# matheusfalcaopinto/triple-hybrid-rag

Hardware: AMD Instinct MI355X
Metric: queries/sec (fused top-10) (higher is better)
Workload: dtype f16 MFMA shortlist scan (f32 accumulate) + f64 rescoring of the f32 rows; 1 GPU; 1000000-doc / 768-d dense-only brute-force cosine top-10 (BASELINE.json configs[1]); pipeline=dense, docs=1000000, dim=768, semantic_top_k=100, fused_top_k=10, shortlist=f16, parallelism=single GPU, world_size_seen=1, rescued_queries=0

## Files before the change

triple-hybrid-rag_amd/_native.py:

```python
from __future__ import annotations

import ctypes as C
import os
from typing import Optional, Tuple

import torch

from . import _build

THR_FLAG_CERTIFIED = 1
THR_FLAG_OVERFLOW = 2
THR_FLAG_EXACT = 4
THR_DENSE_MAX_K = 256
THR_BM25_MAX_TERMS = 32
THR_BM25_MAX_QUERIES = 1 << 20
THR_GRAPH_MAX_SEEDS = 16
THR_RRF_MAX_PER_CHANNEL = 128
THR_TOPK_MAX = 128
THR_SCOPE_MAX_COLS = 8
THR_SCOPE_MAX_PREDS = 4096
THR_SCOPE_MAX_QUERIES = 1 << 20
ABI_VERSION = 9

_lib = None
# ... 92 lines not shown
        except AttributeError as e:
            raise NativeError(f"{path} does not export {name}") from e
        fn.restype, fn.argtypes = res, args
    if lib.thr_abi_version() != ABI_VERSION:
        raise NativeError("libthr_hip.so ABI version mismatch; rebuild")
    _lib = lib
    return lib


def _check(rc: int, what: str) -> None:
    if rc != 0:
        msg = load().thr_error_string(rc).decode()
        raise NativeError(f"{what} failed: {msg} (code {rc})")


def _stream() -> int:
    return torch.cuda.current_stream().cuda_stream


def _dev(t: Optional[torch.Tensor], dtype, name: str, ndim: Optional[int] = None) -> int:
    if t is None:
        return 0
    if not isinstance(t, torch.Tensor) or not t.is_cuda:
        raise NativeError(f"{name}: expected a CUDA(HIP) tensor")
    if t.dtype != dtype:
        raise NativeError(f"{name}: expected dtype {dtype}, got {t.dtype}")
    if not t.is_contiguous():
        raise NativeError(f"{name}: must be contiguous")
    if ndim is not None and t.dim() != ndim:
        raise NativeError(f"{name}: expected {ndim} dims, got {t.dim()}")
    return t.data_ptr()


def device_info() -> Tuple[int, int, str]:
    cus, hbm = C.c_int(0), C.c_int64(0)
    arch = C.create_string_buffer(128)
    torch.cuda.current_device()
    _check(load().thr_device_info(C.byref(cus), C.byref(hbm), arch, 128), "thr_device_info")
    return cus.value, hbm.value, arch.value.decode()


def embed_postproc(full: torch.Tensor, store_dim: int) -> torch.Tensor:
    p = _dev(full, torch.float32, "full", 2)
    n, fd = full.shape
    out = torch.empty((n, min(fd, store_dim)), dtype=torch.float32, device=full.device)
    if n:
        _check(load().thr_embed_postproc(p, n, fd, store_dim, out.data_ptr(), _stream()),
               "thr_embed_postproc")
    return out


def doc_norms(docs: torch.Tensor) -> Tuple[torch.Tensor, torch.Tensor]:
    p = _dev(docs, torch.float32, "docs", 2)
    n, d = docs.shape
    dn = torch.empty(n, dtype=torch.float64, device=docs.device)
    inv = torch.empty(n, dtype=torch.float32, device=docs.device)
    if n:
        _check(load().thr_doc_norms(p, n, d, dn.data_ptr(), inv.data_ptr(), _stream()),
               "thr_doc_norms")
    return dn, inv


def dense_workspace_bytes(n_docs: int, dim: int, n_queries: int, kprime: int) -> int:
    return int(load().thr_dense_workspace_bytes(n_docs, dim, n_queries, kprime))


def _alloc_out(nq: int, k: int, device):
    tile = torch.empty((2, nq, k), dtype=torch.int64, device=device)
    return (tile[0].view(torch.float64), tile[1],
            torch.empty(nq, dtype=torch.int32, device=device),
            torch.empty(nq, dtype=torch.int32, device=device))


def _coll(doc_coll, query_coll, n: int, nq: int):
    if query_coll is None:
        return None, None
    if doc_coll is None:
        raise NativeError("query_coll without doc_coll")
    if doc_coll.shape != (n,) or query_coll.shape != (nq,):
        raise NativeError("doc_coll / query_coll have the wrong length")
    return _dev(doc_coll, torch.int32, "doc_coll", 1), _dev(query_coll, torch.int32, "query_coll", 1)


def dense_topk(docs, dnorm, inv_norm, queries, k: int, kprime: int, id_base: int = 0,
               workspace: Optional[torch.Tensor] = None, doc_coll=None, query_coll=None):
    pd = _dev(docs, torch.float32, "docs", 2)
    n, d = docs.shape
    pq = _dev(queries, torch.float32, "queries", 2)
    nq = queries.shape[0]
    if queries.shape[1] != d:
        raise NativeError(f"queries dim {queries.shape[1]} != docs dim {d}")
    pn = _dev(dnorm, torch.float64, "dnorm", 1)
    pi = _dev(inv_norm, torch.float32, "inv_norm", 1)
    if dnorm.shape[0] != n or inv_norm.shape[0] != n:
        raise NativeError("dnorm / inv_norm length != n_docs")
    need = dense_workspace_bytes(n, d, nq, kprime)
    if workspace is None or workspace.numel() * workspace.element_size() < need:
        workspace = torch.empty(need, dtype=torch.uint8, device=docs.device)
    pw = _dev(workspace, workspace.dtype, "workspace")
    S, I, cnt, flg = _alloc_out(nq, k, docs.device)
    pdc, pqc = _coll(doc_coll, query_coll, n, nq)
    _check(load().thr_dense_topk(pd, pn, pi, n, d, id_base, pq, nq, k, kprime, pdc, pqc, S.data_ptr(),
                                 I.data_ptr(), cnt.data_ptr(), flg.data_ptr(), pw,
                                 workspace.numel() * workspace.element_size(), _stream()),
           "thr_dense_topk")
    return S, I, cnt, flg


def dense_topk_exact(docs, dnorm, queries, k: int, id_base: int = 0, doc_coll=None, query_coll=None):
    pd = _dev(docs, torch.float32, "docs", 2)
    n, d = docs.shape
    pq = _dev(queries, torch.float32, "queries", 2)
    nq = queries.shape[0]
    if queries.shape[1] != d:
        raise NativeError(f"queries dim {queries.shape[1]} != docs dim {d}")
    pn = _dev(dnorm, torch.float64, "dnorm", 1)
    if dnorm.shape[0] != n:
        raise NativeError("dnorm length != n_docs")
    need = int(load().thr_dense_exact_workspace_bytes(n, nq))
    ws = torch.empty(need, dtype=torch.uint8, device=docs.device)
    S, I, cnt, flg = _alloc_out(nq, k, docs.device)
    pdc, pqc = _coll(doc_coll, query_coll, n, nq)
    _check(load().thr_dense_topk_exact(pd, pn, n, d, id_base, pq, nq, k, pdc, pqc, S.data_ptr(),
                                       I.data_ptr(), cnt.data_ptr(), flg.data_ptr(),
                                       ws.data_ptr(), need, _stream()), "thr_dense_topk_exact")
    return S, I, cnt, flg


def dense_scan_probe(docs, inv_norm, queries, workspace: torch.Tensor) -> None:
    pd = _dev(docs, torch.float32, "docs", 2)
    n, d = docs.shape
    pq = _dev(queries, torch.float32, "queries", 2)
    if queries.shape[1] != d or inv_norm.shape[0] != n:
        raise NativeError("probe: shape mismatch")
    pi = _dev(inv_norm, torch.float32, "inv_norm", 1)
    pw = _dev(workspace, workspace.dtype, "workspace")
    _check(load().thr_dense_scan_probe(pd, pi, n, d, pq, queries.shape[0], pw,
                                       workspace.numel() * workspace.element_size(), _stream()),
           "thr_dense_scan_probe")


def dense_f16_query_tile(dim: int, packed: bool, n_queries: int) -> int:
    return int(load().thr_dense_f16_query_tile(dim, 1 if packed else 0, n_queries))


def dense_f16_max_queries(dim: int, packed: bool) -> int:
    return int(load().thr_dense_f16_max_queries(dim, 1 if packed else 0))


def dense_rescue_workspace_bytes(n_queries: int, k: int) -> int:
    return int(load().thr_dense_rescue_workspace_bytes(n_queries, k))


def dense_rescue(docs, dnorm, queries, S, I, cnt, flg, id_base: int = 0,
                 workspace: Optional[torch.Tensor] = None, doc_coll=None, query_coll=None) -> torch.Tensor:
    pd = _dev(docs, torch.float32, "docs", 2)
    pn = _dev(dnorm, torch.float64, "dnorm", 1)
    pq = _dev(queries, torch.float32, "queries", 2)
    n, d = docs.shape
    nq, k = I.shape
    need = int(load().thr_dense_rescue_workspace_bytes(nq, k))
    if workspace is None or workspace.numel() * workspace.element_size() < need:
        workspace = torch.empty(need, dtype=torch.uint8, device=docs.device)
    n_rescued = torch.zeros(1, dtype=torch.int32, device=docs.device)
    pdc, pqc = _coll(doc_coll, query_coll, n, nq)
    _check(load().thr_dense_rescue(pd, pn, n, d, id_base, pq, nq, k, pdc, pqc, S.data_ptr(), I.data_ptr(),
                                   cnt.data_ptr(), flg.data_ptr(), n_rescued.data_ptr(),
                                   workspace.data_ptr(),
                                   workspace.numel() * workspace.element_size(), _stream()),
           "thr_dense_rescue")
    return n_rescued


def dense_quantize_f16(docs: torch.Tensor, keep_copy: bool = True):
    p = _dev(docs, torch.float32, "docs", 2)
    n, d = docs.shape
    d16 = None
    if keep_copy:
        nbytes = int(load().thr_dense_f16_copy_bytes(n, d))
        d16 = torch.empty((nbytes // (2 * d), d), dtype=torch.float16, device=docs.device)
    err = torch.zeros(1, dtype=torch.float32, device=docs.device)
    _check(load().thr_dense_quantize_f16(p, n, d, d16.data_ptr() if keep_copy else None,
                                         err.data_ptr(), _stream()), "thr_dense_quantize_f16")
    return d16, float(err.item())


def dense_quantize_f16_into(docs: torch.Tensor, d16: Optional[torch.Tensor], err: torch.Tensor) -> None:
    p = _dev(docs, torch.float32, "docs", 2)
    n, d = docs.shape
    pe = _dev(err, torch.float32, "err", 1)
    ph = None
    if d16 is not None:
        ph = _dev(d16, torch.float16, "d16", 2)
        if d16.shape[1] != d or d16.numel() * 2 < int(load().thr_dense_f16_copy_bytes(n, d)):
            raise NativeError("dense_quantize_f16_into: the float16 destination is too small")
    if err.numel() != 1:
        raise NativeError("dense_quantize_f16_into: err is one float32")
    _check(load().thr_dense_quantize_f16(p, n, d, ph, pe, _stream()), "thr_dense_quantize_f16")


def dense_f16_layout(dim: int) -> str:
    return f"fragment-major/mfma{32 if os.environ.get('THR_DENSE_MFMA') == '32' else 16}/dim{dim}"


def dense_f16_workspace_bytes(n_docs: int, dim: int, n_queries: int, kprime: int) -> int:
    return int(load().thr_dense_f16_workspace_bytes(n_docs, dim, n_queries, kprime))


def dense_topk_f16(docs, docs16, doc_rel_err: float, dnorm, inv_norm, queries, k: int,
                   kprime: int, id_base: int = 0, workspace: Optional[torch.Tensor] = None,
                   doc_coll=None, query_coll=None):
    pd = _dev(docs, torch.float32, "docs", 2)
    ph = _dev(docs16, torch.float16, "docs16", 2) if docs16 is not None else None
    n, d = docs.shape
    if docs16 is not None and tuple(docs16.shape) != ((n + 31) // 32 * 32, d):
        raise NativeError("docs16 is not the fragment-major copy of docs (thr_dense_quantize_f16)")
    pq = _dev(queries, torch.float32, "queries", 2)
    nq = queries.shape[0]
    if queries.shape[1] != d:
        raise NativeError(f"queries dim {queries.shape[1]} != docs dim {d}")
    pn = _dev(dnorm, torch.float64, "dnorm", 1)
    pi = _dev(inv_norm, torch.float32, "inv_norm", 1)
    if dnorm.shape[0] != n or inv_norm.shape[0] != n:
        raise NativeError("dnorm / inv_norm length != n_docs")
    need = dense_f16_workspace_bytes(n, d, nq, kprime)
    if workspace is None or workspace.numel() * workspace.element_size() < need:
        workspace = torch.empty(need, dtype=torch.uint8, device=docs.device)
    pw = _dev(workspace, workspace.dtype, "workspace")
    S, I, cnt, flg = _alloc_out(nq, k, docs.device)
    pdc, pqc = _coll(doc_coll, query_coll, n, nq)
    _check(load().thr_dense_topk_f16(pd, ph, float(doc_rel_err), pn, pi, n, d, id_base, pq, nq, k,
                                     kprime, pdc, pqc, S.data_ptr(), I.data_ptr(), cnt.data_ptr(),
                                     flg.data_ptr(), pw,
                                     workspace.numel() * workspace.element_size(), _stream()),
           "thr_dense_topk_f16")
    return S, I, cnt, flg


def dense_shortlist_f16(docs, docs16, doc_rel_err: float, inv_norm, queries, kprime: int, m: int,
                        workspace: torch.Tensor, doc_coll=None, query_coll=None) -> torch.Tensor:
    pd = _dev(docs, torch.float32, "docs", 2)
    ph = _dev(docs16, torch.float16, "docs16", 2) if docs16 is not None else None
    n, d = docs.shape
    pq = _dev(queries, torch.float32, "queries", 2)
    nq = queries.shape[0]
    if queries.shape[1] != d or inv_norm.shape[0] != n:
        raise NativeError("shortlist: shape mismatch")
    pi = _dev(inv_norm, torch.float32, "inv_norm", 1)
    need = dense_f16_workspace_bytes(n, d, nq, kprime)
    if workspace.numel() * workspace.element_size() < need:
        raise NativeError("shortlist: workspace smaller than thr_dense_f16_workspace_bytes")
    pw = _dev(workspace, workspace.dtype, "workspace")
    pdc, pqc = _coll(doc_coll, query_coll, n, nq)
    lb = torch.empty((nq, m), dtype=torch.float32, device=docs.device)
    _check(load().thr_dense_shortlist_f16(pd, ph, float(doc_rel_err), pi, n, d, pq, nq, kprime, pdc, pqc,
                                          m, lb.data_ptr(), pw,
                                          workspace.numel() * workspace.element_size(), _stream()),
           "thr_dense_shortlist_f16")
    return lb


def dense_floor(top_lb: torch.Tensor, k: int) -> torch.Tensor:
    p = _dev(top_lb, torch.float32, "top_lb", 3)
    g, nq, m = top_lb.shape
    out = torch.empty(nq, dtype=torch.float32, device=top_lb.device)
    _check(load().thr_dense_floor(p, g, nq, m, k, out.data_ptr(), _stream()), "thr_dense_floor")
    return out


def dense_finish_f16(docs, docs16, doc_rel_err: float, dnorm, inv_norm, queries, k: int, kprime: int,
                     gfloor: Optional[torch.Tensor], id_base: int, workspace: torch.Tensor,
                     doc_coll=None, query_coll=None, lb_all: Optional[torch.Tensor] = None):
    pd = _dev(docs, torch.float32, "docs", 2)
    ph = _dev(docs16, torch.float16, "docs16", 2) if docs16 is not None else None
    n, d = docs.shape
    pq = _dev(queries, torch.float32, "queries", 2)
    nq = queries.shape[0]
    pn = _dev(dnorm, torch.float64, "dnorm", 1)
    pi = _dev(inv_norm, torch.float32, "inv_norm", 1)
    if queries.shape[1] != d or dnorm.shape[0] != n or inv_norm.shape[0] != n:
        raise NativeError("finish: shape mismatch")
    pg = None
    if gfloor is not None:
        pg = _dev(gfloor, torch.float32, "gfloor", 1)
        if gfloor.shape[0] != nq:
            raise NativeError("gfloor: one value per query")
    pl, g, m = None, 0, 0
    if lb_all is not None:
        if gfloor is not None:
            raise NativeError("finish: gfloor or lb_all, not both")
        pl = _dev(lb_all, torch.float32, "lb_all", 3)
        g, nq_l, m = lb_all.shape
        if nq_l != nq:
            raise NativeError("lb_all: [n_shards, nq, m]")
    pw = _dev(workspace, workspace.dtype, "workspace")
    S, I, cnt, flg = _alloc_out(nq, k, docs.device)
    pdc, pqc = _coll(doc_coll, query_coll, n, nq)
    _check(load().thr_dense_finish_f16(pd, ph, float(doc_rel_err), pn, pi, n, d, id_base, pq, nq, k,
                                       kprime, pdc, pqc, pg, pl, g, m, S.data_ptr(), I.data_ptr(),
                                       cnt.data_ptr(), flg.data_ptr(), pw,
                                       workspace.numel() * workspace.element_size(), _stream()),
           "thr_dense_finish_f16")
    return S, I, cnt, flg


def dense_scan_probe_f16(docs, docs16, inv_norm, queries, workspace: torch.Tensor) -> None:
    pd = _dev(docs, torch.float32, "docs", 2)
    ph = _dev(docs16, torch.float16, "docs16", 2) if docs16 is not None else None
    n, d = docs.shape
    pq = _dev(queries, torch.float32, "queries", 2)
    if queries.shape[1] != d or inv_norm.shape[0] != n:
        raise NativeError("probe: shape mismatch")
    pi = _dev(inv_norm, torch.float32, "inv_norm", 1)
    pw = _dev(workspace, workspace.dtype, "workspace")
    _check(load().thr_dense_scan_probe_f16(pd, ph, pi, n, d, pq, queries.shape[0], pw,
                                           workspace.numel() * workspace.element_size(),
                                           _stream()), "thr_dense_scan_probe_f16")
# ... 508 lines not shown
```

triple-hybrid-rag_amd/csrc/dense.hip:

```cpp
#include <stdlib.h>

#include "dense_common.hpp"

namespace thr {

struct DenseKnobs {
    bool forced_q;
    int shape;
    bool forced32;
};
static const DenseKnobs& dense_knobs() {
    static const DenseKnobs knobs = [] {
        DenseKnobs K;
        const char* e = getenv("THR_DENSE_F16");
        K.forced_q = e && e[0] == 'q';
        e = getenv("THR_DENSE_MFMA");
        K.shape = (e && atoi(e) == 32) ? 32 : 16;
        e = getenv("THR_DENSE_QW");
        K.forced32 = e && atoi(e) == 32;
        return K;
    }();
    return knobs;
}

bool qreg_staggered(int dim) { return !dense_knobs().forced_q && dim <= 768; }
int qreg_waves(int dim) { return qreg_staggered(dim) ? 8 : 4; }
int qreg_shape(int) { return dense_knobs().shape; }
int qreg_qw(int dim) {
    return (dim == 1024 && !qreg_staggered(dim) && qreg_shape(dim) == 16 && !dense_knobs().forced32) ? 48 : 32;
}
constexpr int QREG_MAX_SEG = 1024;
int qreg_max_queries(int dim) {
    const int qt = qreg_qw(dim) * qreg_waves(dim);
    const int64_t m = (int64_t)UINT32_MAX / ((int64_t)CAND_CAP * (int64_t)sizeof(Cand));
    return (int)(m / qt * qt);
}


static DensePlan make_plan(void* ws, int64_t n_docs, int n_queries, int kprime, int kind, int dim,
                           bool packed) {
    DensePlan p;
    p.kind = kind;
    p.packed = kind == KIND_F16 && packed;
    p.nq = (kind == KIND_F16 && !p.packed) ? f16_pick_nq(dim) : 1;
    p.row_bits = (kind == KIND_F16 && !p.packed) ? ROW_BITS_F16 : ROW_BITS;
    p.qtile = p.packed ? qreg_qw(dim) * qreg_waves(dim)
              : kind == KIND_F16 ? 32 * p.nq : MF_QT;
    p.ntiles = (n_queries + p.qtile - 1) / p.qtile;
    p.qpad = p.ntiles * p.qtile;
    const int64_t groups = (n_docs + MF_ROWS - 1) / MF_ROWS;
    p.sampled = n_docs > CAND_CAP / 2;
    const int ks_cap = p.packed ? 32 : 64;
    p.ksample = kprime < ks_cap ? kprime : ks_cap;
    double aim = (p.packed ? 2896.0 : 4096.0) * sqrt((double)n_docs / 1.0e6);
    const double aim_lo = 8.0 * kprime < 4096.0 ? 8.0 * kprime : 4096.0;
    aim = aim < aim_lo ? aim_lo : aim > 4096.0 ? 4096.0 : aim;
    int64_t target = (int64_t)((double)n_docs * (double)p.ksample / aim);
    if (target > SAMPLE_MAX) target = SAMPLE_MAX;
    if (target < 4 * (int64_t)p.ksample) target = 4 * (int64_t)p.ksample;
    int64_t sg = (target + MF_ROWS - 1) / MF_ROWS;
    if (sg > groups) sg = groups;
    p.sample_stride = sg > 0 ? groups / sg : 1;
    if (p.sample_stride < 1) p.sample_stride = 1;
    p.sample_groups = p.sampled ? sg : 0;
    p.sample_docs = p.sample_groups * MF_ROWS;
    p.groups = groups;
    p.tile_cap = p.packed ? 1 : p.qtile * (CAND_CAP / 2);
    const size_t qpad = (size_t)p.qpad;
    Arena A{(char*)ws};
    p.tau = A.take<float>(qpad);
    p.qerr = A.take<float>(qpad);
    if (kind != KIND_F16) p.qerr = nullptr;
    p.cnt = A.take<int>(qpad * (p.packed ? QREG_MAX_SEG : 1));
    p.tcnt = A.take<int>(p.ntiles);
    p.cand = A.take<Cand>(qpad * CAND_CAP);
    p.tlist = A.take<Cand>((size_t)p.ntiles * p.tile_cap);
    p.sample = A.take<float>(qpad * (size_t)p.sample_docs);
    p.qfrag = A.take<_Float16>(p.packed ? qpad * (size_t)dim : 0);
    p.sel_rows = A.take<int32_t>(qpad * SEL_BIG_BAND);
    p.sel_meta = A.take<int32_t>(4 * qpad);
    p.total = A.total;
    return p;
}

dim3 scan_grid(int ntiles, int64_t n_row_tiles, int waves, bool* shared_rows, int blocks_per_cu,
               int m_cap) {
    const int cus = num_cus() * blocks_per_cu;
    int64_t m_max = n_row_tiles / (8 * (int64_t)waves);
    if (m_max < 1) m_max = 1;
    if (m_max > m_cap) m_max = m_cap;
    int best_m = 1;
    double best_eff = 0.0;
    for (int m = 1; m <= (int)m_max; ++m) {
        const int64_t g = 8 * (int64_t)m * ntiles;
        const int64_t rounds = (g + cus - 1) / cus;
        const double eff = (double)g / (double)(rounds * cus);
        if (eff > best_eff + 1e-9) {
            best_eff = eff;
            best_m = m;
        }
    }
    *shared_rows = ntiles > 1;
    return dim3((unsigned)(8 * best_m * ntiles), 1u);
}

bool scan_nt(bool shared_rows) { return !shared_rows; }


template <int MODE>
static int launch_scan(const DensePlan& P, const DenseIndex& X, const DenseBatch& B, int* nseg = nullptr) {
    constexpr bool all = MODE == MODE_ALL;
    const int64_t units = all ? P.sample_groups : P.groups, stride = all ? P.sample_stride : 1;
    const float* tau = all ? nullptr : P.tau;
    float* smp = all ? P.sample : nullptr;
    const int64_t ld = all ? P.sample_docs : 0;
    const int32_t* doc_coll = all ? nullptr : X.doc_coll;
    const int32_t* query_coll = all ? nullptr : B.query_coll;
    if (P.packed)
        return launch_scan_f16q<MODE>(X.dim, X.docs16, P.qfrag, P.ntiles, units, stride, tau,
                                      all ? nullptr : P.cnt, all ? nullptr : P.cand, smp, ld, B.st,
                                      nseg, doc_coll, query_coll, B.n_queries);
    int* tcnt = all ? nullptr : P.tcnt;
    Cand* tlist = all ? nullptr : P.tlist;
    const int tile_cap = all ? 0 : P.tile_cap;
    if (P.kind == KIND_F16)
        return launch_scan_f16<MODE>(X.dim, P.nq, X.docs, X.inv_norm, X.n_docs, B.queries, B.n_queries,
                                     P.ntiles, units, stride, tau, tcnt, tlist, tile_cap, smp, ld, B.st,
                                     doc_coll, query_coll);
    return launch_scan_mfma<MODE>(X.dim, X.docs, X.inv_norm, X.n_docs, B.queries, B.n_queries, P.ntiles,
                                  units, stride, tau, tcnt, tlist, tile_cap, smp, ld, B.st, doc_coll,
                                  query_coll);
}

static int dense_pipeline(const DensePlan& P, const DenseIndex& X, const DenseBatch& B,
                          const DensePhase& S) {
    int rc, nseg = 0;
    if (S.phase != PIPE_FINISH) {
        hipError_t e = hipMemsetAsync(P.cnt, 0, (char*)P.cand - (char*)P.cnt, B.st);
        if (e != hipSuccess) return (int)e;
        if (P.packed && (rc = launch_pack_queries(X.dim, B.queries, B.n_queries, P.qpad, P.qfrag, P.qerr, B.st)))
            return rc;
        if (P.sampled && (rc = launch_scan<MODE_ALL>(P, X, B))) return rc;
        if ((rc = launch_threshold(P, X, B))) return rc;
        if ((rc = launch_scan<MODE_FILTER>(P, X, B, &nseg))) return rc;
        if (!P.packed && (rc = launch_bucket(P, B.st))) return rc;
    } else if (P.packed) {
        if ((rc = launch_scan_f16q<MODE_FILTER, true>(X.dim, X.docs16, P.qfrag, P.ntiles, P.groups, 1,
                                                      nullptr, nullptr, nullptr, nullptr, 0, B.st, &nseg)))
            return rc;
    }
    if ((rc = launch_band(P, X, B, S, nseg))) return rc;
    if (S.phase == PIPE_SHORTLIST) return THR_OK;
    return launch_rescore(P, X, B);
}

}

using namespace thr;

extern "C" size_t thr_dense_workspace_bytes(int64_t n_docs, int dim, int n_queries, int kprime) {
    if (n_docs <= 0 || n_queries <= 0) return 0;
    return make_plan(nullptr, n_docs, n_queries, kprime, KIND_F32, dim, false).total;
}

static int dense_args_ok(const void* docs, const void* dnorm, const void* inv_norm,
                         const void* queries, const void* a, const void* b, const void* c,
                         const void* d, const void* ws, int64_t n_docs, int n_queries, int k,
                         int kprime) {
    THR_RETURN_IF(!docs || !dnorm || !inv_norm || !queries || !a || !b || !c || !d || !ws,
                  THR_ERR_INVALID);
    THR_RETURN_IF(n_docs <= 0 || n_queries <= 0 || k <= 0 || kprime < k ||
                      kprime > THR_DENSE_MAX_K,
                  THR_ERR_INVALID);
    return THR_OK;
}

extern "C" int thr_dense_topk(const float* docs, const double* dnorm, const float* inv_norm,
                              int64_t n_docs, int dim, int64_t id_base, const float* queries,
                              int n_queries, int k, int kprime, const int32_t* doc_coll,
                              const int32_t* query_coll, double* out_scores,
                              int64_t* out_ids, int32_t* out_counts, uint32_t* out_flags,
                              void* workspace, size_t workspace_bytes, thr_stream_t stream) {
    clear_status();
    int rc = dense_args_ok(docs, dnorm, inv_norm, queries, out_scores, out_ids, out_counts,
                           out_flags, workspace, n_docs, n_queries, k, kprime);
    if (rc) return rc;
    THR_RETURN_IF((query_coll != nullptr) != (doc_coll != nullptr), THR_ERR_INVALID);
    THR_RETURN_IF(dim <= 0 || dim % CHUNK != 0 || dim / CHUNK > 4, THR_ERR_UNSUPPORTED);
    THR_RETURN_IF(n_docs >= (int64_t)1 << ROW_BITS, THR_ERR_UNSUPPORTED);
    const DensePlan P = make_plan(workspace, n_docs, n_queries, kprime, KIND_F32, dim, false);
    THR_RETURN_IF(workspace_bytes < P.total, THR_ERR_WORKSPACE);
    const DenseIndex X{docs, inv_norm, n_docs, dim, dnorm, id_base, doc_coll};
    const DenseBatch B{queries, n_queries, k, kprime, query_coll, (hipStream_t)stream,
                       out_scores, out_ids, out_counts, out_flags};
    return dense_pipeline(P, X, B, DensePhase{});
}

extern "C" size_t thr_dense_f16_workspace_bytes(int64_t n_docs, int dim, int n_queries,
                                                int kprime) {
    if (n_docs <= 0 || n_queries <= 0) return 0;
    const size_t a = make_plan(nullptr, n_docs, n_queries, kprime, KIND_F16, dim, false).total;
    const size_t b = make_plan(nullptr, n_docs, n_queries, kprime, KIND_F16, dim, true).total;
    return a > b ? a : b;
}

extern "C" int thr_dense_f16_max_queries(int dim, int packed) {
    if (dim != 512 && dim != 768 && dim != 1024) return 0;
    return packed ? qreg_max_queries(dim) : INT32_MAX;
}

extern "C" int thr_dense_f16_query_tile(int dim, int packed, int n_queries) {
    if (dim != 512 && dim != 768 && dim != 1024) return 0;
    (void)n_queries;
    return packed ? qreg_qw(dim) * qreg_waves(dim) : 32 * f16_pick_nq(dim);
}

extern "C" size_t thr_dense_f16_copy_bytes(int64_t n_docs, int dim) {
    if (n_docs <= 0 || dim <= 0) return 0;
    return sizeof(_Float16) * (size_t)((n_docs + 31) / 32 * 32) * (size_t)dim;
}

extern "C" int thr_dense_quantize_f16(const float* docs, int64_t n_docs, int dim, uint16_t* docs16,
                                      float* max_rel_err, thr_stream_t stream) {
    clear_status();
    THR_RETURN_IF(!docs || !max_rel_err || n_docs <= 0 || dim <= 0, THR_ERR_INVALID);
    THR_RETURN_IF(dim % 64 != 0, THR_ERR_UNSUPPORTED);
    hipStream_t st = (hipStream_t)stream;
    hipError_t e = hipMemsetAsync(max_rel_err, 0, sizeof(float), st);
    if (e != hipSuccess) return (int)e;
    return launch_quantize_f16(docs, n_docs, dim, reinterpret_cast<_Float16*>(docs16),
                               reinterpret_cast<unsigned int*>(max_rel_err), st);
}

static int f16_args_ok(const float* docs, const uint16_t* docs16, double doc_rel_err, int64_t n_docs,
                       int dim, int n_queries, const int32_t* doc_coll, const int32_t* query_coll) {
    (void)docs;
    THR_RETURN_IF((query_coll != nullptr) != (doc_coll != nullptr), THR_ERR_INVALID);
    THR_RETURN_IF(!(doc_rel_err >= 0.0) || !(doc_rel_err < 1.0), THR_ERR_INVALID);
    THR_RETURN_IF(dim != 512 && dim != 768 && dim != 1024, THR_ERR_UNSUPPORTED);
    THR_RETURN_IF(n_docs >= (int64_t)1 << ROW_BITS_F16, THR_ERR_UNSUPPORTED);
    THR_RETURN_IF(docs16 != nullptr && n_queries > qreg_max_queries(dim), THR_ERR_UNSUPPORTED);
    return THR_OK;
}


extern "C" int thr_dense_topk_f16(const float* docs, const uint16_t* docs16, double doc_rel_err,
                                  const double* dnorm, const float* inv_norm, int64_t n_docs,
                                  int dim, int64_t id_base, const float* queries, int n_queries,
                                  int k, int kprime, const int32_t* doc_coll,
                                  const int32_t* query_coll, double* out_scores, int64_t* out_ids,
                                  int32_t* out_counts, uint32_t* out_flags, void* workspace,
                                  size_t workspace_bytes, thr_stream_t stream) {
    clear_status();
    int rc = dense_args_ok(docs, dnorm, inv_norm, queries, out_scores, out_ids, out_counts,
                           out_flags, workspace, n_docs, n_queries, k, kprime);
    if (rc) return rc;
    if ((rc = f16_args_ok(docs, docs16, doc_rel_err, n_docs, dim, n_queries, doc_coll, query_coll))) return rc;
    const DensePlan P = make_plan(workspace, n_docs, n_queries, kprime, KIND_F16, dim, docs16 != nullptr);
    THR_RETURN_IF(workspace_bytes < P.total, THR_ERR_WORKSPACE);
    const DenseIndex X{docs, inv_norm, n_docs, dim, dnorm, id_base, doc_coll,
                       reinterpret_cast<const _Float16*>(docs16), doc_rel_err};
    const DenseBatch B{queries, n_queries, k, kprime, query_coll, (hipStream_t)stream,
                       out_scores, out_ids, out_counts, out_flags};
    return dense_pipeline(P, X, B, DensePhase{});
}

extern "C" int thr_dense_shortlist_f16(const float* docs, const uint16_t* docs16, double doc_rel_err,
                                       const float* inv_norm, int64_t n_docs, int dim,
                                       const float* queries, int n_queries, int kprime,
                                       const int32_t* doc_coll, const int32_t* query_coll, int m,
                                       float* top_lb, void* workspace, size_t workspace_bytes,
                                       thr_stream_t stream) {
    clear_status();
    THR_RETURN_IF(!docs || !inv_norm || !queries || !top_lb || !workspace, THR_ERR_INVALID);
    THR_RETURN_IF(n_docs <= 0 || n_queries <= 0 || kprime <= 0 || kprime > THR_DENSE_MAX_K || m <= 0 ||
                      m > THR_DENSE_MAX_K,
                  THR_ERR_INVALID);
    int rc = f16_args_ok(docs, docs16, doc_rel_err, n_docs, dim, n_queries, doc_coll, query_coll);
    if (rc) return rc;
    const DensePlan P = make_plan(workspace, n_docs, n_queries, kprime, KIND_F16, dim, docs16 != nullptr);
    THR_RETURN_IF(workspace_bytes < P.total, THR_ERR_WORKSPACE);
    const DenseIndex X{docs, inv_norm, n_docs, dim, nullptr, 0, doc_coll,
                       reinterpret_cast<const _Float16*>(docs16), doc_rel_err};
    const DenseBatch B{queries, n_queries, 0, kprime, query_coll, (hipStream_t)stream};
    return dense_pipeline(P, X, B, DensePhase{PIPE_SHORTLIST, top_lb, m});
}

extern "C" int thr_dense_finish_f16(const float* docs, const uint16_t* docs16, double doc_rel_err,
                                    const double* dnorm, const float* inv_norm, int64_t n_docs,
                                    int dim, int64_t id_base, const float* queries, int n_queries,
                                    int k, int kprime, const int32_t* doc_coll,
                                    const int32_t* query_coll, const float* gfloor,
// ... 81 lines not shown
```

triple-hybrid-rag_amd/csrc/rrf.hip:

```cpp
#include "thr_common.hpp"

namespace thr {

constexpr int RRF_THREADS = 128;
constexpr int RRF_MAXC = THR_RRF_MAX_PER_CHANNEL;
constexpr int RRF_SLOTS = 512;

__device__ __forceinline__ int last_rank(const int64_t* l, int n, int64_t id) {
    int r = 0;
    for (int j = 0; j < n; ++j)
        if (l[j] == id) r = j + 1;
    return r;
}
__device__ __forceinline__ bool seen_before(const int64_t* l, int i, int64_t id) {
    for (int j = 0; j < i; ++j)
        if (l[j] == id) return true;
    return false;
}

constexpr int RRF_RAG2 = 0, RRF_STANDALONE = 1, RRF_TWO = 2;
__device__ __forceinline__ int occurrences(const int64_t* l, int n, int64_t id) {
    int c = 0;
    for (int j = 0; j < n; ++j) c += l[j] == id ? 1 : 0;
    return c;
}

template <int MODE>
__global__ __launch_bounds__(RRF_THREADS) void rrf_fuse_kernel(
    const int64_t* __restrict__ lex, int n_lex, const int64_t* __restrict__ sem, int n_sem,
    const int64_t* __restrict__ gra, int n_gra, double w_lex, double w_sem, double w_gra, int rrf_k,
    int top_k, int64_t* __restrict__ out_ids, double* __restrict__ out_scores,
    int32_t* __restrict__ out_ranks, int32_t* __restrict__ out_counts) {
    static_assert(RRF_THREADS == RRF_MAXC && RRF_THREADS == 2 * WAVE, "one thread per position");
    __shared__ int64_t L[3][RRF_MAXC];
    __shared__ int len[3];
    __shared__ int wave_new[3][2];
    __shared__ double s_s[RRF_SLOTS];
    __shared__ int64_t c_id[RRF_SLOTS];
    __shared__ int c_rank[RRF_SLOTS][3];
    __shared__ int order[RRF_SLOTS];

    const int q = blockIdx.x, t = threadIdx.x, lane = t & 63, wave = t >> 6;
    const int64_t* src[3] = {lex, sem, gra};
    const int width[3] = {lex ? n_lex : 0, sem ? n_sem : 0, gra ? n_gra : 0};
    if (t < 3) len[t] = width[t];
    __syncthreads();
    for (int ch = 0; ch < 3; ++ch) {
        const int64_t id = t < width[ch] ? src[ch][(int64_t)q * width[ch] + t] : -1;
        L[ch][t] = id;
        if (t < width[ch] && id < 0) atomicMin(&len[ch], t);
    }
    __syncthreads();

    bool nw[3];
    int within[3];
    for (int ch = 0; ch < 3; ++ch) {
        nw[ch] = false;
        if (t < len[ch]) {
            const int64_t id = L[ch][t];
            nw[ch] = !seen_before(L[ch], t, id);
            for (int e = 0; e < ch && nw[ch]; ++e)
                if (last_rank(L[e], len[e], id)) nw[ch] = false;
        }
        const uint64_t m = __ballot(nw[ch]);
        within[ch] = __popcll(m & ((1ull << lane) - 1ull));
        if (lane == 0) wave_new[ch][wave] = __popcll(m);
    }
    __syncthreads();
    int base = 0, n = 0;
    for (int ch = 0; ch < 3; ++ch) {
        const int here = base + (wave ? wave_new[ch][0] : 0) + within[ch];
        base += wave_new[ch][0] + wave_new[ch][1];
        if (!nw[ch]) continue;
        const int64_t id = L[ch][t];
        const int lr = last_rank(L[0], len[0], id);
        const int sr = last_rank(L[1], len[1], id);
        const int gr = last_rank(L[2], len[2], id);
        double score = 0.0;
        if (MODE == RRF_RAG2) {
            if (lr) score = __dadd_rn(score, __ddiv_rn(w_lex, (double)(rrf_k + lr)));
            if (sr) score = __dadd_rn(score, __ddiv_rn(w_sem, (double)(rrf_k + sr)));
            if (gr) score = __dadd_rn(score, __ddiv_rn(w_gra, (double)(rrf_k + gr)));
        } else {
            const double w[3] = {w_lex, w_sem, w_gra};
            const int rk[3] = {lr, sr, gr};
#pragma unroll
            for (int c = 0; c < 3; ++c)
                if (rk[c]) {
                    const double v = __dmul_rn(w[c], __ddiv_rn(1.0, (double)(rrf_k + rk[c])));
                    const int reps = (MODE == RRF_TWO && c == 0) ? 1 : occurrences(L[c], len[c], id);
                    for (int r = 0; r < reps; ++r) score = __dadd_rn(score, v);
                }
        }
        c_id[here] = id;
        c_rank[here][0] = lr;
        c_rank[here][1] = sr;
        c_rank[here][2] = gr;
        s_s[here] = score;
    }
    n = base;
    __syncthreads();
    for (int p = t; p < n; p += RRF_THREADS) {
        const double ms = s_s[p];
        int rank = 0;
        for (int j = 0; j < n; ++j) {
            const double o = s_s[j];
            rank += (o > ms || (o == ms && j < p)) ? 1 : 0;
        }
        order[rank] = p;
    }
    __syncthreads();
    for (int i = t; i < top_k; i += RRF_THREADS) {
        const bool ok = i < n;
        const int p = ok ? order[i] : 0;
        out_ids[(int64_t)q * top_k + i] = ok ? c_id[p] : -1;
        out_scores[(int64_t)q * top_k + i] = ok ? s_s[p] : -INFINITY;
        if (out_ranks)
            for (int c = 0; c < 3; ++c)
                out_ranks[((int64_t)q * top_k + i) * 3 + c] = ok ? c_rank[p][c] : 0;
    }
    if (t == 0) out_counts[q] = n < top_k ? n : top_k;
}

__global__ __launch_bounds__(RRF_THREADS) void rerank_order_kernel(
    const float* __restrict__ scores, int n_lists, int64_t list_stride,
    const int64_t* __restrict__ ids, const int32_t* __restrict__ counts, int n, int top_k,
    int64_t* __restrict__ out_ids, double* __restrict__ out_scores, int32_t* __restrict__ out_counts) {
    __shared__ double s_s[RRF_SLOTS];
    __shared__ int order[RRF_SLOTS];
    const int q = blockIdx.x, t = threadIdx.x;
    int cnt = counts ? counts[q] : n;
    cnt = cnt < n ? cnt : n;
    for (int p = t; p < cnt; p += RRF_THREADS) {
        float best = -INFINITY;
        for (int l = 0; l < n_lists; ++l) best = fmaxf(best, scores[(int64_t)l * list_stride + (int64_t)q * n + p]);
        s_s[p] = best > -INFINITY ? (double)best : 0.0;
    }
    __syncthreads();
    for (int p = t; p < cnt; p += RRF_THREADS) {
        const double ms = s_s[p];
        int rank = 0;
        for (int j = 0; j < cnt; ++j) {
            const double o = s_s[j];
            rank += (o > ms || (o == ms && j < p)) ? 1 : 0;
        }
        order[rank] = p;
    }
    __syncthreads();
    for (int i = t; i < top_k; i += RRF_THREADS) {
        const bool ok = i < cnt;
        const int p = ok ? order[i] : 0;
        out_ids[(int64_t)q * top_k + i] = ok ? ids[(int64_t)q * n + p] : -1;
        out_scores[(int64_t)q * top_k + i] = ok ? s_s[p] : -INFINITY;
    }
    if (t == 0) out_counts[q] = cnt < top_k ? cnt : top_k;
}

__global__ __launch_bounds__(RRF_THREADS) void fuse_post_kernel(
    const int64_t* __restrict__ ids, const double* __restrict__ scores,
    const int32_t* __restrict__ ranks, const int32_t* __restrict__ counts, int n,
    const double* __restrict__ lex_s, int n_lex, const double* __restrict__ sem_s, int n_sem,
    const double* __restrict__ gra_s, int n_gra, double safety_threshold, int denoise,
    double quantile, int normalize, int top_k, int64_t* __restrict__ out_ids,
    double* __restrict__ out_scores, int32_t* __restrict__ out_counts) {
    __shared__ double s_s[2][RRF_SLOTS];
    __shared__ int64_t s_id[2][RRF_SLOTS];
    __shared__ int wave_cnt[2];
    __shared__ double red[2][2];
    const int q = blockIdx.x, t = threadIdx.x, lane = t & 63, wave = t >> 6;
    int cnt = counts ? counts[q] : n;
    cnt = cnt < n ? cnt : n;
    auto compact = [&](int from, int m, auto keep) -> int {
        int base = 0;
        for (int b0 = 0; b0 < m; b0 += RRF_THREADS) {
            const int i = b0 + t;
            const bool k = i < m && keep(i);
            const uint64_t bal = __ballot(k);
            if (lane == 0) wave_cnt[wave] = __popcll(bal);
            __syncthreads();
            const int at = base + (wave ? wave_cnt[0] : 0) + __popcll(bal & ((1ull << lane) - 1ull));
            if (k) {
                s_s[from ^ 1][at] = s_s[from][i];
                s_id[from ^ 1][at] = s_id[from][i];
            }
            base += wave_cnt[0] + wave_cnt[1];
            __syncthreads();
        }
        return base;
    };
    const double* chs[3] = {lex_s, sem_s, gra_s};
    const int chw[3] = {n_lex, n_sem, n_gra};
    for (int i = t; i < cnt; i += RRF_THREADS) {
        s_s[0][i] = scores[(int64_t)q * n + i];
        s_id[0][i] = ids[(int64_t)q * n + i];
    }
    __syncthreads();
    int m = cnt, cur = 0;
    if (safety_threshold > 0.0 && ranks) {
        m = compact(0, cnt, [&](int i) {
            double best = 0.0;
            for (int c = 0; c < 3; ++c) {
                const int r = ranks[((int64_t)q * n + i) * 3 + c];
                if (r > 0 && chs[c]) {
                    const double v = chs[c][(int64_t)q * chw[c] + r - 1];
                    best = v > best ? v : best;
                }
            }
            return best >= safety_threshold;
        });
        cur = 1;
    }
    if (denoise && m >= 3) {
        const double v = __dmul_rn((double)(m - 1), quantile);
        int prev = (int)floor(v);
        prev = prev < 0 ? 0 : prev > m - 1 ? m - 1 : prev;
        const int next = prev + 1 > m - 1 ? m - 1 : prev + 1;
        const double g = __dsub_rn(v, (double)prev);
        const double a = s_s[cur][m - 1 - prev], bb = s_s[cur][m - 1 - next];
        const double diff = __dsub_rn(bb, a);
        const double cut = g >= 0.5 ? __dsub_rn(bb, __dmul_rn(diff, __dsub_rn(1.0, g)))
                                    : __dadd_rn(a, __dmul_rn(diff, g));
        __syncthreads();
        const int from = cur;
        m = compact(from, m, [&](int i) { return s_s[from][i] >= cut; });
        cur ^= 1;
    }
    if (top_k > 0 && m > top_k) m = top_k;
    double lo = 0.0, hi = 0.0;
    if (normalize && m > 0) {
        double mn = INFINITY, mx = -INFINITY;
        for (int i = t; i < m; i += RRF_THREADS) {
            const double v = s_s[cur][i];
            mn = v < mn ? v : mn;
            mx = v > mx ? v : mx;
        }
        for (int o = 32; o > 0; o >>= 1) {
            const double a = __shfl_xor(mn, o, WAVE), b2 = __shfl_xor(mx, o, WAVE);
            mn = a < mn ? a : mn;
            mx = b2 > mx ? b2 : mx;
        }
        if (lane == 0) {
            red[0][wave] = mn;
            red[1][wave] = mx;
        }
        __syncthreads();
        lo = red[0][0] < red[0][1] ? red[0][0] : red[0][1];
        hi = red[1][0] > red[1][1] ? red[1][0] : red[1][1];
    }
    for (int i = t; i < n; i += RRF_THREADS) {
        const bool ok = i < m;
        double v = ok ? s_s[cur][i] : -INFINITY;
        if (ok && normalize) v = hi == lo ? 1.0 : __ddiv_rn(__dsub_rn(v, lo), __dsub_rn(hi, lo));
        out_scores[(int64_t)q * n + i] = v;
        out_ids[(int64_t)q * n + i] = ok ? s_id[cur][i] : -1;
    }
    if (t == 0) out_counts[q] = m;
}

}

using namespace thr;

extern "C" int thr_rerank_order(const float* scores, int n_lists, int64_t list_stride,
                                const int64_t* ids, const int32_t* counts, int n_queries, int n,
                                int top_k, int64_t* out_ids, double* out_scores,
                                int32_t* out_counts, thr_stream_t stream) {
    clear_status();
    THR_RETURN_IF(!scores || !ids || !out_ids || !out_scores || !out_counts, THR_ERR_INVALID);
    THR_RETURN_IF(n_queries <= 0 || n_lists <= 0 || n <= 0 || n > RRF_SLOTS || top_k <= 0 || top_k > n,
                  THR_ERR_INVALID);
    if (list_stride == 0) list_stride = (int64_t)n_queries * n;
    THR_RETURN_IF(list_stride < (int64_t)n_queries * n, THR_ERR_INVALID);
    hipLaunchKernelGGL(rerank_order_kernel, dim3(n_queries), dim3(RRF_THREADS), 0, (hipStream_t)stream,
                       scores, n_lists, list_stride, ids, counts, n, top_k, out_ids, out_scores,
                       out_counts);
    return launch_status();
}

extern "C" int thr_rrf_fuse(const int64_t* lex_ids, int n_lex, const int64_t* sem_ids, int n_sem,
                            const int64_t* graph_ids, int n_graph, int n_queries, double w_lex,
                            double w_sem, double w_graph, int rrf_k, int top_k, int64_t* out_ids,
                            double* out_scores, int32_t* out_ranks, int32_t* out_counts,
                            thr_stream_t stream) {
    clear_status();
    THR_RETURN_IF(!out_ids || !out_scores || !out_counts, THR_ERR_INVALID);
    THR_RETURN_IF(n_queries <= 0 || top_k <= 0 || top_k > RRF_SLOTS || rrf_k < 0, THR_ERR_INVALID);
    THR_RETURN_IF(n_lex < 0 || n_sem < 0 || n_graph < 0 || n_lex > RRF_MAXC || n_sem > RRF_MAXC ||
                      n_graph > RRF_MAXC,
                  THR_ERR_INVALID);
    THR_RETURN_IF((!lex_ids || !n_lex) && (!sem_ids || !n_sem) && (!graph_ids || !n_graph),
                  THR_ERR_INVALID);
    hipLaunchKernelGGL(rrf_fuse_kernel<RRF_RAG2>, dim3(n_queries), dim3(RRF_THREADS), 0, (hipStream_t)stream,
                       n_lex ? lex_ids : nullptr, n_lex, n_sem ? sem_ids : nullptr, n_sem,
                       n_graph ? graph_ids : nullptr, n_graph, w_lex, w_sem, w_graph, rrf_k, top_k,
                       out_ids, out_scores, out_ranks, out_counts);
    return launch_status();
}

extern "C" int thr_rrf_fuse_standalone(const int64_t* lex_ids, int n_lex, const int64_t* sem_ids,
                                       int n_sem, const int64_t* graph_ids, int n_graph,
                                       int n_queries, double w_lex, double w_sem, double w_graph,
                                       int two_channels, int top_k, int64_t* out_ids,
                                       double* out_scores, int32_t* out_ranks, int32_t* out_counts,
                                       thr_stream_t stream) {
    clear_status();
    THR_RETURN_IF(!out_ids || !out_scores || !out_counts, THR_ERR_INVALID);
    THR_RETURN_IF(n_queries <= 0 || top_k <= 0 || top_k > RRF_SLOTS, THR_ERR_INVALID);
    THR_RETURN_IF(n_lex < 0 || n_sem < 0 || n_graph < 0 || n_lex > RRF_MAXC || n_sem > RRF_MAXC ||
                      n_graph > RRF_MAXC,
                  THR_ERR_INVALID);
    THR_RETURN_IF((!lex_ids || !n_lex) && (!sem_ids || !n_sem) && (!graph_ids || !n_graph),
                  THR_ERR_INVALID);
    THR_RETURN_IF(two_channels && graph_ids && n_graph, THR_ERR_INVALID);
    const int rrf_k = 60;
#define THR_RRF_LAUNCH(MODE)                                                                        \
    hipLaunchKernelGGL(rrf_fuse_kernel<MODE>, dim3(n_queries), dim3(RRF_THREADS), 0, (hipStream_t)stream, \
                       n_lex ? lex_ids : nullptr, n_lex, n_sem ? sem_ids : nullptr, n_sem,          \
                       n_graph ? graph_ids : nullptr, n_graph, w_lex, w_sem, w_graph, rrf_k, top_k, \
                       out_ids, out_scores, out_ranks, out_counts)
    if (two_channels) THR_RRF_LAUNCH(RRF_TWO);
    else THR_RRF_LAUNCH(RRF_STANDALONE);
#undef THR_RRF_LAUNCH
    return launch_status();
}

extern "C" int thr_fuse_post(const int64_t* ids, const double* scores, const int32_t* ranks,
                             const int32_t* counts, int n_queries, int n, const double* lex_scores,
                             int n_lex, const double* sem_scores, int n_sem,
                             const double* graph_scores, int n_graph, double safety_threshold,
                             int denoise, double quantile, int normalize, int top_k,
                             int64_t* out_ids, double* out_scores, int32_t* out_counts,
                             thr_stream_t stream) {
    clear_status();
    THR_RETURN_IF(!ids || !scores || !out_ids || !out_scores || !out_counts, THR_ERR_INVALID);
    THR_RETURN_IF(n_queries <= 0 || n <= 0 || n > RRF_SLOTS || top_k < 0, THR_ERR_INVALID);
    THR_RETURN_IF(safety_threshold > 0.0 && !ranks, THR_ERR_INVALID);
    THR_RETURN_IF(denoise && !(quantile >= 0.0 && quantile <= 1.0), THR_ERR_INVALID);
    THR_RETURN_IF(n_lex < 0 || n_sem < 0 || n_graph < 0, THR_ERR_INVALID);
    hipLaunchKernelGGL(fuse_post_kernel, dim3(n_queries), dim3(RRF_THREADS), 0, (hipStream_t)stream, ids,
                       scores, ranks, counts, n, lex_scores, n_lex, sem_scores, n_sem, graph_scores,
                       n_graph, safety_threshold, denoise, quantile, normalize, top_k, out_ids,
                       out_scores, out_counts);
    return launch_status();
}
```

Baseline: 733,200 queries/s.

## Skip counter memset for packed path, pool rescue counters, add single-channel RRF fast path

Three unrelated changes. The Python rescue wrapper now hands out slices of a pooled zeroed int32 buffer instead of allocating a new zero tensor per call. The dense pipeline skips the candidate-count memset when the packed f16 path is used, unless THR_DENSE_CLEAR=1. The RRF fuse kernel gains a fast path that, when only one channel is present with non-negative weight and no duplicates, writes ranks and scores directly without the general dedup and merge. Risks: the pooled counters are never re-zeroed and wrap after 4096 uses, and skipping the memset assumes the packed kernels clear or never read those counters.

```diff
diff --git a/triple-hybrid-rag_amd/_native.py b/triple-hybrid-rag_amd/_native.py
--- a/triple-hybrid-rag_amd/_native.py
+++ b/triple-hybrid-rag_amd/_native.py
@@ -268,6 +268,18 @@
     return int(load().thr_dense_rescue_workspace_bytes(n_queries, k))
 
 
+_ZEROS = {}
+
+
+def _zero_counter(device) -> torch.Tensor:
+    key = (device, torch.cuda.current_stream(device).cuda_stream)
+    slot = _ZEROS.get(key)
+    if slot is None or slot[1] >= slot[0].numel():
+        slot = _ZEROS[key] = [torch.zeros(4096, dtype=torch.int32, device=device), 0]
+    slot[1] += 1
+    return slot[0][slot[1] - 1:slot[1]]
+
+
 def dense_rescue(docs, dnorm, queries, S, I, cnt, flg, id_base: int = 0,
                  workspace: Optional[torch.Tensor] = None, doc_coll=None, query_coll=None) -> torch.Tensor:
     pd = _dev(docs, torch.float32, "docs", 2)
@@ -278,7 +290,7 @@
     need = int(load().thr_dense_rescue_workspace_bytes(nq, k))
     if workspace is None or workspace.numel() * workspace.element_size() < need:
         workspace = torch.empty(need, dtype=torch.uint8, device=docs.device)
-    n_rescued = torch.zeros(1, dtype=torch.int32, device=docs.device)
+    n_rescued = _zero_counter(docs.device)
     pdc, pqc = _coll(doc_coll, query_coll, n, nq)
     _check(load().thr_dense_rescue(pd, pn, n, d, id_base, pq, nq, k, pdc, pqc, S.data_ptr(), I.data_ptr(),
                                    cnt.data_ptr(), flg.data_ptr(), n_rescued.data_ptr(),
diff --git a/triple-hybrid-rag_amd/csrc/dense.hip b/triple-hybrid-rag_amd/csrc/dense.hip
--- a/triple-hybrid-rag_amd/csrc/dense.hip
+++ b/triple-hybrid-rag_amd/csrc/dense.hip
@@ -8,6 +8,7 @@
     bool forced_q;
     int shape;
     bool forced32;
+    bool clear_cnt;
 };
 static const DenseKnobs& dense_knobs() {
     static const DenseKnobs knobs = [] {
@@ -18,6 +19,8 @@
         K.shape = (e && atoi(e) == 32) ? 32 : 16;
         e = getenv("THR_DENSE_QW");
         K.forced32 = e && atoi(e) == 32;
+        e = getenv("THR_DENSE_CLEAR");
+        K.clear_cnt = e && atoi(e) == 1;
         return K;
     }();
     return knobs;
@@ -136,8 +139,10 @@
                           const DensePhase& S) {
     int rc, nseg = 0;
     if (S.phase != PIPE_FINISH) {
-        hipError_t e = hipMemsetAsync(P.cnt, 0, (char*)P.cand - (char*)P.cnt, B.st);
-        if (e != hipSuccess) return (int)e;
+        if (!P.packed || dense_knobs().clear_cnt) {
+            hipError_t e = hipMemsetAsync(P.cnt, 0, (char*)P.cand - (char*)P.cnt, B.st);
+            if (e != hipSuccess) return (int)e;
+        }
         if (P.packed && (rc = launch_pack_queries(X.dim, B.queries, B.n_queries, P.qpad, P.qfrag, P.qerr, B.st)))
             return rc;
         if (P.sampled && (rc = launch_scan<MODE_ALL>(P, X, B))) return rc;
diff --git a/triple-hybrid-rag_amd/csrc/rrf.hip b/triple-hybrid-rag_amd/csrc/rrf.hip
--- a/triple-hybrid-rag_amd/csrc/rrf.hip
+++ b/triple-hybrid-rag_amd/csrc/rrf.hip
@@ -1,3 +1,5 @@
+#include <stdlib.h>
+
 #include "thr_common.hpp"
 
 namespace thr {
@@ -30,7 +32,7 @@
     const int64_t* __restrict__ lex, int n_lex, const int64_t* __restrict__ sem, int n_sem,
     const int64_t* __restrict__ gra, int n_gra, double w_lex, double w_sem, double w_gra, int rrf_k,
     int top_k, int64_t* __restrict__ out_ids, double* __restrict__ out_scores,
-    int32_t* __restrict__ out_ranks, int32_t* __restrict__ out_counts) {
+    int32_t* __restrict__ out_ranks, int32_t* __restrict__ out_counts, int fast) {
     static_assert(RRF_THREADS == RRF_MAXC && RRF_THREADS == 2 * WAVE, "one thread per position");
     __shared__ int64_t L[3][RRF_MAXC];
     __shared__ int len[3];
@@ -52,30 +54,7 @@
     }
     __syncthreads();
 
-    bool nw[3];
-    int within[3];
-    for (int ch = 0; ch < 3; ++ch) {
-        nw[ch] = false;
-        if (t < len[ch]) {
-            const int64_t id = L[ch][t];
-            nw[ch] = !seen_before(L[ch], t, id);
-            for (int e = 0; e < ch && nw[ch]; ++e)
-                if (last_rank(L[e], len[e], id)) nw[ch] = false;
-        }
-        const uint64_t m = __ballot(nw[ch]);
-        within[ch] = __popcll(m & ((1ull << lane) - 1ull));
-        if (lane == 0) wave_new[ch][wave] = __popcll(m);
-    }
-    __syncthreads();
-    int base = 0, n = 0;
-    for (int ch = 0; ch < 3; ++ch) {
-        const int here = base + (wave ? wave_new[ch][0] : 0) + within[ch];
-        base += wave_new[ch][0] + wave_new[ch][1];
-        if (!nw[ch]) continue;
-        const int64_t id = L[ch][t];
-        const int lr = last_rank(L[0], len[0], id);
-        const int sr = last_rank(L[1], len[1], id);
-        const int gr = last_rank(L[2], len[2], id);
+    auto fused_score = [&](int64_t id, int lr, int sr, int gr) {
         double score = 0.0;
         if (MODE == RRF_RAG2) {
             if (lr) score = __dadd_rn(score, __ddiv_rn(w_lex, (double)(rrf_k + lr)));
@@ -92,6 +71,58 @@
                     for (int r = 0; r < reps; ++r) score = __dadd_rn(score, v);
                 }
         }
+        return score;
+    };
+    {
+        const int one = len[0] ? (len[1] || len[2] ? -1 : 0) : len[1] ? (len[2] ? -1 : 1) : 2;
+        const double w1 = one == 0 ? w_lex : one == 1 ? w_sem : w_gra;
+        if (fast && one >= 0 && w1 >= 0.0) {
+            const int n1 = len[one];
+            const int64_t id = L[one][t];
+            bool dup = false;
+            for (int j = 0; j < n1; ++j) dup |= j < t && L[one][j] == id;
+            if (!__syncthreads_or(dup && t < n1)) {
+                for (int i = t; i < top_k; i += RRF_THREADS) {
+                    const bool ok = i < n1;
+                    const int r = i + 1;
+                    out_ids[(int64_t)q * top_k + i] = ok ? L[one][i] : -1;
+                    out_scores[(int64_t)q * top_k + i] =
+                        ok ? fused_score(L[one][i], one == 0 ? r : 0, one == 1 ? r : 0, one == 2 ? r : 0) : -INFINITY;
+                    if (out_ranks)
+                        for (int c = 0; c < 3; ++c)
+                            out_ranks[((int64_t)q * top_k + i) * 3 + c] = (ok && c == one) ? r : 0;
+                }
+                if (t == 0) out_counts[q] = n1 < top_k ? n1 : top_k;
+                return;
+            }
+        }
+    }
+
+    bool nw[3];
+    int within[3];
+    for (int ch = 0; ch < 3; ++ch) {
+        nw[ch] = false;
+        if (t < len[ch]) {
+            const int64_t id = L[ch][t];
+            nw[ch] = !seen_before(L[ch], t, id);
+            for (int e = 0; e < ch && nw[ch]; ++e)
+                if (last_rank(L[e], len[e], id)) nw[ch] = false;
+        }
+        const uint64_t m = __ballot(nw[ch]);
+        within[ch] = __popcll(m & ((1ull << lane) - 1ull));
+        if (lane == 0) wave_new[ch][wave] = __popcll(m);
+    }
+    __syncthreads();
+    int base = 0, n = 0;
+    for (int ch = 0; ch < 3; ++ch) {
+        const int here = base + (wave ? wave_new[ch][0] : 0) + within[ch];
+        base += wave_new[ch][0] + wave_new[ch][1];
+        if (!nw[ch]) continue;
+        const int64_t id = L[ch][t];
+        const int lr = last_rank(L[0], len[0], id);
+        const int sr = last_rank(L[1], len[1], id);
+        const int gr = last_rank(L[2], len[2], id);
+        const double score = fused_score(id, lr, sr, gr);
         c_id[here] = id;
         c_rank[here][0] = lr;
         c_rank[here][1] = sr;
@@ -257,6 +288,14 @@
     if (t == 0) out_counts[q] = m;
 }
 
+static int rrf_fast() {
+    static const int on = [] {
+        const char* e = getenv("THR_RRF_FAST");
+        return (e && e[0] == '0') ? 0 : 1;
+    }();
+    return on;
+}
+
 }
 
 using namespace thr;
@@ -293,7 +332,7 @@
     hipLaunchKernelGGL(rrf_fuse_kernel<RRF_RAG2>, dim3(n_queries), dim3(RRF_THREADS), 0, (hipStream_t)stream,
                        n_lex ? lex_ids : nullptr, n_lex, n_sem ? sem_ids : nullptr, n_sem,
                        n_graph ? graph_ids : nullptr, n_graph, w_lex, w_sem, w_graph, rrf_k, top_k,
-                       out_ids, out_scores, out_ranks, out_counts);
+                       out_ids, out_scores, out_ranks, out_counts, rrf_fast());
     return launch_status();
 }
 
@@ -317,7 +356,7 @@
     hipLaunchKernelGGL(rrf_fuse_kernel<MODE>, dim3(n_queries), dim3(RRF_THREADS), 0, (hipStream_t)stream, \
                        n_lex ? lex_ids : nullptr, n_lex, n_sem ? sem_ids : nullptr, n_sem,          \
                        n_graph ? graph_ids : nullptr, n_graph, w_lex, w_sem, w_graph, rrf_k, top_k, \
-                       out_ids, out_scores, out_ranks, out_counts)
+                       out_ids, out_scores, out_ranks, out_counts, rrf_fast())
     if (two_channels) THR_RRF_LAUNCH(RRF_TWO);
     else THR_RRF_LAUNCH(RRF_STANDALONE);
 #undef THR_RRF_LAUNCH
```

New measurement: 735,600 queries/s (median of 4 runs). No clear change (+0.3%).
